# cb-geo/2d-lbm-dem

Measured on AMD Instinct MI355X. Metric: MLUPS (D2Q9 collide+stream, coupled LBM-DEM step) on 4096^2 / 50k grains, higher is better.
Workload: dtype f64; 1 GPU; 4096x4096 D2Q9 MRT + 50000 grains (synthetic row packing, seed 1234); lx=4096, ly=4096, grains=50000, npDEM=12, step=1 fluid step + npDEM DEM sub-steps (+ Verlet rebuild every 100 DEM steps), force_kernel=parity, fused_launches_reading_one_map=1996, settle_steps=40, decomposition=none

## Files before the change

2d-lbm-dem_amd/csrc/lbm_fused.hip:

```cpp


#include "lbm_march.h"
#include <type_traits>

#ifdef LBMDEM_AB
void launch_march3_ab(int which, int lx_template, const real* fin, real* fout, const int* obst_old, const int* obst_new,
                      const LatticeView& L, const GrainFluidView& G, const ForceSlots& S, int nstrips, int nwork, int remap,
                      int seg_rows, int seg_stride, int grid, hipStream_t st);
#endif

namespace {

template <int TX, int TY>
struct TileCtx {
  const Tile<TX, TY>& T;
  const LatticeView& L;
  const GrainFluidView& G;
  int px, py, gx, gy;
  __device__ __forceinline__ real own(int q) const { return T.F(q, px, py); }
  __device__ __forceinline__ real in(int d) const { return T.F(OPPq(d), px + EXq(d), py + EYq(d)); }
  __device__ __forceinline__ int o_own() const { return T.O(px, py); }
  __device__ __forceinline__ int o_nb(int d) const { return T.O(px + EXq(d), py + EYq(d)); }
  __device__ __forceinline__ bool act_nb(int d) const {
    return T.active(L, G, px + EXq(d), py + EYq(d), gx + EXq(d), gy + EYq(d));
  }
  __device__ __forceinline__ GP gp_nb(int d) const { return load_gp(G, o_nb(d)); }
};

template <int TX, int TY>
__global__ __launch_bounds__(256) void k_collide_stream(const real* __restrict__ fin,
                                                        real* __restrict__ fout,
                                                        const int* __restrict__ ob_old,
                                                        const int* __restrict__ ob_new, LatticeView L,
                                                        GrainFluidView G, int tiles_y, int ntiles,
                                                        int xcd_remap) {
  LBMDEM_GATE(L.gate);
  using TT = Tile<TX, TY>;
  __shared__ real sF[9 * TT::RX * TT::RY];
  __shared__ int sO[TT::OX * TT::OY];
  TT T{sF, sO};
  const int tid = threadIdx.x;
  int t = blockIdx.x;
  if (xcd_remap) {
    const int per = gridDim.x >> 3;
    t = (t & 7) * per + (t >> 3);
  }
  if (t >= ntiles) return;
  const int ty0 = (t % tiles_y) * TY;
  const int txl0 = L.xo0 + (t / tiles_y) * TX;

  for (int k = tid; k < TT::OX * TT::OY; k += 256) {
    const int ox = k / TT::OY, oy = k % TT::OY;
    const int xl = txl0 - 2 + ox, y = ty0 - 2 + oy;
    int v = L.n;
    if (xl >= 0 && xl < L.nxl && y >= 0 && y < L.ly) v = ob_new[(long)xl * L.sy + y];
    sO[k] = v;
  }
  __syncthreads();

  for (int k = tid; k < TT::RX * TT::RY; k += 256) {
    const int rx = k / TT::RY, ry = k % TT::RY;
    const int xl = txl0 - 1 + rx, y = ty0 - 1 + ry;
    if (xl < 0 || xl >= L.nxl || y < 0 || y >= L.ly) continue;
    const int gx = L.gx0 + xl;
    const long node = (long)xl * L.sy + y;
    const bool interior = gx >= 1 && gx <= L.lx - 2 && y >= 1 && y <= L.ly - 2;
    real f[9];
    const int oo = interior ? ob_old[node] : -1;
    if (oo != -1) {
      grain_equilibrium(L, load_gp(G, oo), gx, y, f);
    } else {
#pragma unroll
      for (int q = 0; q < 9; ++q) f[q] = fin[fidx(q, node)];
    }
    if (interior && sO[(rx + 1) * TT::OY + (ry + 1)] == -1) mrt_collide(L, f);
#pragma unroll
    for (int q = 0; q < 9; ++q) sF[(q * TT::RX + rx) * TT::RY + ry] = f[q];
  }
  __syncthreads();

  for (int k = tid; k < TX * TY; k += 256) {
    const int px = k / TY, py = k % TY;
    const int xl = txl0 + px, gy = ty0 + py;
    if (xl >= L.xo1 || gy >= L.ly) continue;
    const int gx = L.gx0 + xl;
    const long node = (long)xl * L.sy + gy;
    const TileCtx<TX, TY> C{T, L, G, px, py, gx, gy};
    fout[fidx(0, node)] = T.F(0, px, py);
    fout[fidx(1, node)] = pull_one<1>(C, L, G, gx, gy);
    fout[fidx(2, node)] = pull_one<2>(C, L, G, gx, gy);
    fout[fidx(3, node)] = pull_one<3>(C, L, G, gx, gy);
    fout[fidx(4, node)] = pull_one<4>(C, L, G, gx, gy);
    fout[fidx(5, node)] = pull_one<5>(C, L, G, gx, gy);
    fout[fidx(6, node)] = pull_one<6>(C, L, G, gx, gy);
    fout[fidx(7, node)] = pull_one<7>(C, L, G, gx, gy);
    fout[fidx(8, node)] = pull_one<8>(C, L, G, gx, gy);
  }
}

struct MarchPlan {
  int nlev, band_rows, chunk;
  int seg[4];
  int off[4];
  int first[5];
};

constexpr int LINK_SLOTS = 64;

template <int WW, bool CHG, bool EDGE>
__device__ __forceinline__ void march_item(const real* __restrict__ fin, real* __restrict__ fout,
                                           const int* __restrict__ ob_old, const int* __restrict__ ob_new,
                                           const LatticeView& L, const LatticeView& Lk, const GrainFluidView& G,
                                           const ForceSlots& S, const ObstChange& CH, int strip, int xs, int xe,
                                           const RecRing ring,
                                           real* const pay, int* const desc, int lane, int w) {
  (void)w;
  constexpr int OFF = (64 - WW) / 2;
  const int y = strip * WW - OFF + lane;
  const bool yin = !EDGE || (y >= 0 && y < L.ly);
  const bool writer = lane >= OFF && lane < OFF + WW && yin;
  const bool deep_y = !EDGE || (strip * WW >= 2 && strip * WW + WW - 1 <= L.ly - 3);

  auto row_ok = [&](int xl) { return !EDGE || (yin && xl >= 0 && xl < L.nxl); };
  const int ycl = !EDGE ? y : (y < 0 ? 0 : (y >= L.ly ? L.ly - 1 : y));
  unsigned long long cm = ~0ull;
  const int row0 = __builtin_amdgcn_readfirstlane(xs - 2 < 0 ? 0 : xs - 2);
  const int frow = L.sy * 9 * (int)sizeof(real), irow = L.sy * 4;
  const __amdgpu_buffer_rsrc_t fin_rs = make_rs(fin + (long)row0 * L.sy * 9, (long)(L.nxl - row0) * frow);
  const __amdgpu_buffer_rsrc_t fout_rs = make_rs(fout + (long)row0 * L.sy * 9, (long)(L.nxl - row0) * frow);
  const __amdgpu_buffer_rsrc_t id_rs = make_rs(ob_new + (long)row0 * L.sy, (long)(L.nxl - row0) * irow);
  const __amdgpu_buffer_rsrc_t old_rs = make_rs(ob_old + (long)row0 * L.sy, (long)(L.nxl - row0) * irow);
  const int fcol = fcol_bytes(ycl), icol = ycl * 4;
  auto rel_row = [&](int xl) { return (xl < 0 ? 0 : (xl >= L.nxl ? L.nxl - 1 : xl)) - row0; };
  if (CHG) {
    const int r0 = xs - 1, first = r0 < 0 ? 0 : r0;
    const unsigned* wp = CH.bits + (long)strip * CH.words + (first >> 5);
    const unsigned w0 = __builtin_amdgcn_readfirstlane(wp[0]), w1 = __builtin_amdgcn_readfirstlane(wp[1]);
    const unsigned w2 = __builtin_amdgcn_readfirstlane(wp[2]);
    const int sh = __builtin_amdgcn_readfirstlane(first & 31);
    cm = (unsigned long long)w0 | ((unsigned long long)w1 << 32);
    if (sh) cm = (cm >> sh) | ((unsigned long long)w2 << (64 - sh));
    if (r0 < 0) cm <<= 1;
  }
  auto load_old = [&](int xl, int same) -> int {
    if (!CHG) return __builtin_amdgcn_raw_buffer_load_b32(old_rs, icol, rel_row(xl) * irow, 0);
    const int keep = (cm & 1ull) ? 0 : -1;
    cm = (cm >> 1) | (1ull << 63);
    const int v = __builtin_amdgcn_raw_buffer_load_b32(old_rs, (rel_row(xl) * irow + icol) | (keep & (int)0x80000000), 0, 0);
    return v | (same & keep);
  };
  auto load_id = [&](int xl) -> int {
    const int v = __builtin_amdgcn_raw_buffer_load_b32(id_rs, icol, rel_row(xl) * irow, 0);
    if (!EDGE) return v;
    return (xl >= 0 && xl < L.nxl && ycl == y) ? v : L.n;
  };
  auto load_raw = [&](int xl, real (&raw)[9]) {
    const int so = rel_row(xl) * frow;
    raw[0] = buf_load_real<0 * F_QBYTES>(fin_rs, fcol, so); raw[1] = buf_load_real<1 * F_QBYTES>(fin_rs, fcol, so);
    raw[2] = buf_load_real<2 * F_QBYTES>(fin_rs, fcol, so); raw[3] = buf_load_real<3 * F_QBYTES>(fin_rs, fcol, so);
    raw[4] = buf_load_real<4 * F_QBYTES>(fin_rs, fcol, so); raw[5] = buf_load_real<5 * F_QBYTES>(fin_rs, fcol, so);
    raw[6] = buf_load_real<6 * F_QBYTES>(fin_rs, fcol, so); raw[7] = buf_load_real<7 * F_QBYTES>(fin_rs, fcol, so);
    raw[8] = buf_load_real<8 * F_QBYTES>(fin_rs, fcol, so);
  };
  auto interior = [&](int xl) {
    const int gx = L.gx0 + xl;
    return !EDGE || (row_ok(xl) && gx >= 1 && gx <= L.lx - 2 && y >= 1 && y <= L.ly - 2);
  };
  auto make_fstar = [&](int xl, real (&f)[9], int oo, const GPv& g, int on) {
    const bool in = interior(xl);
    if (in && oo != -1) grain_equilibrium(L, g, L.gx0 + xl, y, f);
    if (in && on == -1) mrt_collide(L, f);
  };
  auto grain_rec = [&](int id) { return load_gp(G, (id < 0 || id >= L.n) ? 0 : id); };
  auto reinit_rec = [&](int id) { return load_gpv(G, (id < 0 || id >= L.n) ? 0 : id); };

  real Fm[9], F0[9], Fp[9], bufA[9], bufB[9];

  const int iA = load_id(xs - 2);
  int iB = load_id(xs - 1);
  int iC = load_id(xs);
  int iD = load_id(xs + 1);
  int iE = load_id(xs + 2);
  {
    int oo = load_old(xs - 1, iB);
    load_raw(xs - 1, Fm);
    make_fstar(xs - 1, Fm, oo, reinit_rec(oo), iB);
    oo = load_old(xs, iC);
    load_raw(xs, F0);
    make_fstar(xs, F0, oo, reinit_rec(oo), iC);
  }
  ring.put(xs - 1, lane, grain_rec(iB), iB);
  ring.put(xs, lane, grain_rec(iC), iC);
  ring.put(xs + 1, lane, grain_rec(iD), iD);
  ring.put(xs + 2, lane, grain_rec(iE), iE);
  int inext = load_id(xs + 3);
  int oo1 = load_old(xs + 1, iD);
  int oo2 = load_old(xs + 2, iE);
  GP rec_next = grain_rec(inext);
  GPv gv_next = ring.getv(xs + 1, lane);
  load_raw(xs + 1, bufA);
  load_raw(xs + 2, bufB);
  auto sol_of = [&](int c) -> lmask { return __ballot(c != -1); };
  auto hmax_of = [&](int c) { const int m = dpp_up1(c), p = dpp_dn1(c), t = m > c ? m : c; return t > p ? t : p; };
  auto act_of = [&](lmask sa, lmask sb, lmask sc, int hma, int hmb, int hmc, int a, int b, int c, int xl, int ycol) -> lmask {
    const lmask enclosed = sb & m_enclosed(sa, sb, sc);
    lmask act = sb & ~enclosed;
    const int t = hma > hmb ? hma : hmb;
    const lmask rare = __ballot((t > hmc ? t : hmc) > b) & enclosed;
    if (rare != 0) {
      const bool on = node_active(L, G, ids3_of(a), ids3_of(b), ids3_of(c), L.gx0 + xl, ycol, [&] { return ring.get(xl, lane); });
      act |= __ballot(on) & rare;
    }
    return act;
  };
  lmask solB = sol_of(iB), solC = sol_of(iC), solD = sol_of(iD), solE = sol_of(iE);
  int hmC = hmax_of(iC), hmD = hmax_of(iD), hmE = hmax_of(iE);
  lmask actM = act_of(sol_of(iA), solB, solC, hmax_of(iA), hmax_of(iB), hmC, iA, iB, iC, xs - 1, y);
  lmask act0 = act_of(solB, solC, solD, hmax_of(iB), hmC, hmD, iB, iC, iD, xs, y);
  const lmask wmask = EDGE ? __ballot(writer) : (((lmask)1 << WW) - 1) << OFF;

  auto iterate = [&](int x, real (&buf)[9]) {
#pragma unroll
    for (int q = 0; q < 9; ++q) Fp[q] = buf[q];
    {
      const bool in = interior(x + 1), re = in && oo1 != -1, moved = re && oo1 != iD;
      GPv g = gv_next;
      asm volatile("" : "+v"(g.x1), "+v"(g.x2), "+v"(g.v1), "+v"(g.v2), "+v"(g.v3));
      if (__ballot(moved) != 0) {
        if (moved) g = reinit_rec(oo1);
      }
      if (re) grain_equilibrium(Lk, g, L.gx0 + x + 1, y, Fp);
      if (in && iD == -1) mrt_collide(Lk, Fp);
    }
    const int iF = inext;
    oo1 = oo2;
    inext = load_id(x + 4);
    oo2 = load_old(x + 3, iF);
    __builtin_amdgcn_sched_barrier(0);
    load_raw(x + 3 < xe ? x + 3 : xe, buf);
    __builtin_amdgcn_sched_barrier(0);
    int y_act = y;
    asm volatile("" : "+v"(y_act));
    const lmask actP = act_of(solC, solD, solE, hmC, hmD, hmE, iC, iD, iE, x + 1, y_act);

    real Fo[9], In[9];
#pragma unroll
    for (int q = 0; q < 9; ++q) Fo[q] = F0[q];
    In[0] = 0.0;
    In[2] = Fm[6];
    In[6] = Fp[2];
    In[1] = shfl_dn1z(Fm[5]);
    In[8] = shfl_dn1z(F0[4]);
    In[7] = shfl_dn1z(Fp[3]);
    In[3] = shfl_up1z(Fm[7]);
    In[4] = shfl_up1z(F0[8]);
    In[5] = shfl_up1z(Fp[1]);
    {
      const int gx = L.gx0 + x;
      const int so_row = (x - row0) * frow;
      const bool deep = !EDGE || (deep_y && gx >= 2 && gx <= L.lx - 3);
      const lmask wm = x < xe ? wmask : 0;
#define MARCH_SRC(Q) m_at<-EYq(Q)>(MARCH_ROW(-EXq(Q), solB, solC, solD))
#define MARCH_LINK(Q) (wm & ~solC & MARCH_SRC(Q))
#define MARCH_HAZ(Q) (Q <= 4 ? MARCH_LINK(Q) & m_at<EYq(Q)>(MARCH_ROW(EXq(Q), solB, solC, solD)) : 0)
#define MARCH_RESET(Q) (solC & MARCH_SRC(Q) & m_at<-EYq(Q)>(MARCH_ROW(-EXq(Q), actM, act0, actP)))
      unsigned ibb = 0, nnm = 0, hzm = 0;
      int T = 0;
      if (deep) {
        T = __popcll(MARCH_LINK(1)) + __popcll(MARCH_LINK(2)) + __popcll(MARCH_LINK(3)) + __popcll(MARCH_LINK(4)) +
            __popcll(MARCH_LINK(5)) + __popcll(MARCH_LINK(6)) + __popcll(MARCH_LINK(7)) + __popcll(MARCH_LINK(8));
      } else if constexpr (EDGE) {
        RegCtx C;
        C.ring = ring;
        C.row = x;
        C.lane = lane;
#pragma unroll
        for (int q = 0; q < 9; ++q) { C.Fo[q] = Fo[q]; C.In[q] = In[q]; }
        const Ids3 b3 = ids3_of(iB), c3 = ids3_of(iC), d3 = ids3_of(iD);
        C.o0 = iC;
        C.onb[0] = 0;
        C.onb[1] = b3.p; C.onb[2] = b3.c; C.onb[3] = b3.m; C.onb[4] = c3.m;
        C.onb[5] = d3.m; C.onb[6] = d3.c; C.onb[7] = d3.p; C.onb[8] = c3.p;
        C.act = 0;
#define MARCH_ACTBIT(D) C.act |= lane_of(m_at<EYq(D)>(MARCH_ROW(EXq(D), actM, act0, actP))) ? 1u << D : 0u;
        MARCH_ACTBIT(1) MARCH_ACTBIT(2) MARCH_ACTBIT(3) MARCH_ACTBIT(4) MARCH_ACTBIT(5) MARCH_ACTBIT(6) MARCH_ACTBIT(7) MARCH_ACTBIT(8)
#undef MARCH_ACTBIT
        if (writer && x < xe) classify_store_row<true>(C, L, gx, y, fout, fbase_xy(L, x, y), ibb, nnm, hzm);
#pragma unroll
        for (int q = 1; q < 9; ++q) T += __popcll(__ballot((ibb >> q) & 1u));
      }
      const bool merged = deep && T <= LINK_SLOTS;
      auto store_row = [&](auto with_results) {
        if (lane_of(wm)) {
          buf_store_real<0>(Fo[0], fout_rs, fcol, so_row);
          real res[9];
          if constexpr (decltype(with_results)::value) {
            int before = 0;
#define MARCH_RES(Q)                                                                               \
            {                                                                                      \
              const lmask b = MARCH_LINK(Q);                                                       \
              res[Q] = pay[((before + (int)mbcnt(b)) & (LINK_SLOTS - 1)) * 4];                     \
              before += __popcll(b);                                                               \
            }
            MARCH_RES(1) MARCH_RES(2) MARCH_RES(3) MARCH_RES(4) MARCH_RES(5) MARCH_RES(6) MARCH_RES(7) MARCH_RES(8)
#undef MARCH_RES
          }
#define MARCH_STORE(Q)                                                                             \
          {                                                                                        \
            real v = lane_of(MARCH_RESET(Q)) ? Wq(Q) : In[OPPq(Q)];                                \
            if constexpr (decltype(with_results)::value) v = lane_of(MARCH_LINK(Q)) ? res[Q] : v;  \
            buf_store_real<Q * F_QBYTES>(v, fout_rs, fcol, so_row);                                \
          }
          MARCH_STORE(1) MARCH_STORE(2) MARCH_STORE(3) MARCH_STORE(4) MARCH_STORE(5) MARCH_STORE(6) MARCH_STORE(7) MARCH_STORE(8)
#undef MARCH_STORE
        }
      };
      if (deep && !merged) store_row(std::false_type{});
      for (int base = 0; base < T; base += LINK_SLOTS) {
        int before = 0;
        if (deep) {
#define MARCH_COMPACT(Q)                                                                           \
          {                                                                                        \
            const lmask b = MARCH_LINK(Q);                                                         \
            const int t = before + (int)mbcnt(b) - base;                                           \
            before += __popcll(b);                                                                 \
            if (lane_of(b) && (unsigned)t < (unsigned)LINK_SLOTS) {                                \
              desc[t] = lane | (Q << 8) | (1 << 12) | (lane_of(MARCH_HAZ(Q)) ? 1 << 13 : 0);       \
              pay[t * 4 + 0] = Fo[OPPq(Q)];                                                        \
              pay[t * 4 + 1] = Fo[Q];                                                              \
              pay[t * 4 + 2] = In[Q];                                                              \
              pay[t * 4 + 3] = In[OPPq(Q)];                                                        \
            }                                                                                      \
          }
          MARCH_COMPACT(1) MARCH_COMPACT(2) MARCH_COMPACT(3) MARCH_COMPACT(4)
          MARCH_COMPACT(5) MARCH_COMPACT(6) MARCH_COMPACT(7) MARCH_COMPACT(8)
#undef MARCH_COMPACT
        } else if constexpr (EDGE) {
#pragma unroll
          for (int q = 1; q < 9; ++q) {
            const lmask b = __ballot((ibb >> q) & 1u);
            const int t = before + (int)mbcnt(b) - base;
            before += __popcll(b);
            if (((ibb >> q) & 1u) && (unsigned)t < (unsigned)LINK_SLOTS) {
              desc[t] = lane | (q << 8) | (((nnm >> q) & 1u) << 12) | (((hzm >> q) & 1u) << 13);
              pay[t * 4 + 0] = Fo[OPPq(q)];
              pay[t * 4 + 1] = Fo[q];
              pay[t * 4 + 2] = In[q];
              pay[t * 4 + 3] = In[OPPq(q)];
            }
          }
        }
        __builtin_amdgcn_wave_barrier();
        if (base + lane < T) {
          const int d = desc[lane];
          const int src = d & 63;
          RtLink k;
          k.q = (d >> 8) & 15;
          k.gx = gx;
          k.gy = y - lane + src;
          k.own_qo = pay[lane * 4 + 0];
          k.own_q = pay[lane * 4 + 1];
          k.in_q = pay[lane * 4 + 2];
          k.in_qo = pay[lane * 4 + 3];
          k.nn_int = (d >> 12) & 1;
          k.hazard = (d >> 13) & 1;
          const int ex = (k.q >= 1 && k.q <= 3) ? -1 : ((k.q >= 5 && k.q <= 7) ? 1 : 0);
          const int ey = (k.q == 1 || k.q >= 7) ? 1 : ((k.q >= 3 && k.q <= 5) ? -1 : 0);
          const GP gS = ring.get(x - ex, src - ey);
          const int owner = ring.get_id(x - ex, src - ey);
          const real out = ibb_eval_rt(Lk, k, Lk.wc_diag, Lk.wc_axis, gS, [&] { return ring.get(x + ex, src + ey); });
          if (merged) pay[lane * 4] = out;
          else buf_store_real<0>(out, fout_rs, fcol_bytes(k.gy) + k.q * F_QBYTES, so_row);
          if (S.tab != nullptr) {
            const int rel = slot_line(k.gx - ex, k.gy - ey, ex, ey, gS.xc, gS.yc) + S.half;
            if ((unsigned)rel < (unsigned)S.spd)
              S.tab[((long)owner * 8 + (k.q - 1)) * S.spd + rel] = k.own_qo + out;
          }
        }
        __builtin_amdgcn_wave_barrier();
      }
      if (merged) {
        if (T > 0) store_row(std::true_type{});
        else store_row(std::false_type{});
      }
#undef MARCH_RESET
#undef MARCH_HAZ
#undef MARCH_LINK
#undef MARCH_SRC
    }
    ring.put(x + 3, lane, rec_next, iF);
    rec_next = grain_rec(inext);
    gv_next = ring.getv(x + 2, lane);
#pragma unroll
    for (int q = 0; q < 9; ++q) { Fm[q] = F0[q]; F0[q] = Fp[q]; }
    iB = iC; iC = iD; iD = iE; iE = iF;
    solB = solC; solC = solD; solD = solE; solE = sol_of(iF);
    hmC = hmD; hmD = hmE; hmE = hmax_of(iF);
    actM = act0; act0 = actP;
  };

  for (int x = xs; x < xe; x += 2) {
    iterate(x, bufA);
    iterate(x + 1, bufB);
  }
}

constexpr int WPB = 4;

template <int LX, int MINW, int WW, bool CHG = false>
__global__ __launch_bounds__(64 * WPB, MINW) void k_cs_march(const real* __restrict__ fin, real* __restrict__ fout,
                                                  const int* __restrict__ ob_old,
                                                  const int* __restrict__ ob_new, LatticeView L,
                                                  GrainFluidView G, ForceSlots S, int nstrips, int nwork,
                                                  int xcd_remap, int seg_rows, int seg_stride, MarchPlan P, ObstChange CH) {
  LBMDEM_GATE(L.gate);
  const int lane = threadIdx.x & 63;
  int blk = blockIdx.x;
  int w, strip, xs, rows_per_wave;
  if (LX == 0 && P.nlev > 0) {
    const int band = blk & 7, local = (blk >> 3) * WPB + (threadIdx.x >> 6);
    if (local >= P.first[P.nlev]) return;
    int l = 0;
#pragma unroll
    for (int k = 1; k < 4; ++k)
      if (k < P.nlev && local >= P.first[k]) l = k;
    const int j = local - P.first[l], sg = j / nstrips;
    strip = j - sg * nstrips;
    rows_per_wave = P.seg[l];
    const int v = P.off[l] + sg * rows_per_wave, c = v / P.chunk;
    xs = L.xo0 + (c * 8 + band) * P.chunk + (v - c * P.chunk);
    if (xs >= L.xo1) return;
    w = band * P.first[P.nlev] + local;
  } else {
    if (xcd_remap) {
      const int per = gridDim.x >> 3;
      blk = (blk & 7) * per + (blk >> 3);
    }
    w = blk * WPB + (threadIdx.x >> 6);
    if (w >= nwork) return;
    const int seg = w / nstrips;
    strip = w - seg * nstrips;
    rows_per_wave = LX > 0 ? LX : seg_rows;
    xs = L.xo0 + seg * seg_stride;
  }
  strip = __builtin_amdgcn_readfirstlane(strip);
  xs = __builtin_amdgcn_readfirstlane(xs);
  const int xe = __builtin_amdgcn_readfirstlane(xs + rows_per_wave < L.xo1 ? xs + rows_per_wave : L.xo1);
  __shared__ real2 sRec[WPB * REC_RING * 4 * 64];
  __shared__ int sRid[WPB * REC_RING * 64];
  const RecRing ring{sRec + (threadIdx.x >> 6) * (REC_RING * 4 * 64), sRid + (threadIdx.x >> 6) * (REC_RING * 64)};
  __shared__ real sPay[WPB * LINK_SLOTS * 4];
  __shared__ int sDesc[WPB * LINK_SLOTS];
  real* const pay = sPay + (threadIdx.x >> 6) * (LINK_SLOTS * 4);
  int* const desc = sDesc + (threadIdx.x >> 6) * LINK_SLOTS;
  __shared__ LatticeView sLat[WPB];
  LatticeView* const Lk = sLat + (threadIdx.x >> 6);
  if (lane == 0) *Lk = L;
  __builtin_amdgcn_wave_barrier();
  constexpr int OFF = (64 - WW) / 2;
  const int y_lo = strip * WW - OFF;
  const bool inner = y_lo >= 1 && y_lo + 63 <= L.ly - 2 && L.gx0 + xs >= 2 && L.gx0 + xe <= L.lx - 2 && xs >= 2 &&
                     xe + 2 <= L.nxl;
  if (inner) march_item<WW, CHG, false>(fin, fout, ob_old, ob_new, L, *Lk, G, S, CH, strip, xs, xe, ring, pay, desc, lane, w);
  else march_item<WW, CHG, true>(fin, fout, ob_old, ob_new, L, *Lk, G, S, CH, strip, xs, xe, ring, pay, desc, lane, w);
}

}


template <int TX, int TY>
static void launch_cs(const real* fin, real* fout, const int* obst_old, const int* obst_new,
                      const LatticeView& L, const GrainFluidView& G, int remap, hipStream_t st) {
  const int rows = L.xo1 - L.xo0;
  const int tiles_y = (L.ly + TY - 1) / TY, tiles_x = (rows + TX - 1) / TX;
  const int ntiles = tiles_y * tiles_x;
  const int grid = remap ? ((ntiles + 7) / 8) * 8 : ntiles;
  hipLaunchKernelGGL((k_collide_stream<TX, TY>), dim3(grid), dim3(256), 0, st, fin, fout, obst_old, obst_new,
                     L, G, tiles_y, ntiles, remap);
}

static int march_segment_rows(int rows, int nstrips) {
  const int resident = 256 * 2 * 4;
  int nseg = (2 * resident + nstrips - 1) / nstrips;
  if (nseg < 1) nseg = 1;
  int seg_rows = rows / nseg;
  seg_rows &= ~1;
  if (seg_rows < 8) seg_rows = 8;
  if (seg_rows > 32) seg_rows = 32;
  return seg_rows;
}

static MarchPlan march_plan(int rows, int nstrips, int main_seg, const int (*tail)[2], int ntail, int chunk) {
  MarchPlan P{};
  if (rows < 8 * (main_seg + 64)) return P;
  if (chunk <= 0) chunk = 1 << 30;
  int band_rows = (((rows + 7) / 8) + 7) & ~7;
  if (chunk < band_rows) band_rows = (band_rows + chunk - 1) / chunk * chunk;
  else chunk = band_rows;
  P.chunk = chunk;
  int tail_rows = 0;
  for (int k = 0; k < ntail; ++k) tail_rows += tail[k][1];
  if (band_rows - tail_rows < main_seg) return P;
  const int main_rows = (band_rows - tail_rows) / main_seg * main_seg;
  int rem = band_rows - tail_rows - main_rows;
  P.band_rows = band_rows;
  int off = 0, first = 0, lev = 0;
  bool fits = true;
  auto add = [&](int seg, int r) {
    if (r <= 0) return;
    if (chunk % seg != 0 || off % seg != 0) fits = false;
    P.seg[lev] = seg; P.off[lev] = off; P.first[lev] = first;
    off += r; first += r / seg * nstrips; ++lev;
  };
  add(main_seg, main_rows);
  for (int k = 0; k < ntail; ++k) {
    int r = tail[k][1];
    const int seg = tail[k][0];
    const int take = k + 1 < ntail ? rem / seg * seg : rem;
    r += take; rem -= take;
    add(seg, r);
  }
  if (rem != 0 || !fits) return MarchPlan{};
  P.nlev = lev;
  P.first[lev] = first;
  return P;
}

static constexpr bool plan_level_ok(int seg, int rows) { return seg >= 8 && seg % 8 == 0 && rows % seg == 0; }

static MarchPlan product_plan(int rows, int nstrips, int seg_rows) {
  if (seg_rows < 32) return MarchPlan{};
  constexpr int main_seg = 64, ntail = 3, chunk = 64;
  static constexpr int tail[ntail][2] = {{32, 64}, {16, 64}, {8, 64}};
  static_assert(plan_level_ok(main_seg, chunk), "a chunk of a band holds whole main segments");
  static_assert(plan_level_ok(tail[0][0], tail[0][1]) && plan_level_ok(tail[1][0], tail[1][1]) &&
                    plan_level_ok(tail[2][0], tail[2][1]),
                "every tail level is cut into whole segments");
  return march_plan(rows, nstrips, main_seg, tail, ntail, chunk);
}

#ifdef LBMDEM_AB
static int cs_variant() {
  static int v = -1;
  if (v < 0) {
    const char* e = getenv("LBMDEM_CS_VARIANT");
    v = e ? atoi(e) : 25;
  }
  return v;
}
static int march_kernel() {
  static const int v = getenv("LBMDEM_MARCH") ? atoi(getenv("LBMDEM_MARCH")) : 2;
  return v;
}
#endif

constexpr int MARCH_WW = 60;

template <int LX, int MINW, int WW = MARCH_WW>
static void launch_march(const real* fin, real* fout, const int* obst_old, const int* obst_new,
                         const LatticeView& L, const GrainFluidView& G, const ForceSlots& S, int remap,
                         hipStream_t st, ObstChange chg = ObstChange{nullptr, 0, 0, 0}) {
  const int rows = L.xo1 - L.xo0;
  const int nstrips = (L.ly + WW - 1) / WW;
  if (chg.ww != WW || chg.off != (64 - WW) / 2) chg = ObstChange{nullptr, 0, 0, 0};
  int seg_rows = LX;
  if (LX == 0) {
    seg_rows = march_segment_rows(rows, nstrips);
  }
  const int nseg = (rows + seg_rows - 1) / seg_rows;
  int nwork = nstrips * nseg;
  int grid = (nwork + WPB - 1) / WPB;
  if (remap) grid = ((grid + 7) / 8) * 8;
  MarchPlan P{};
  if (LX == 0 && remap) P = product_plan(rows, nstrips, seg_rows);
  if (P.nlev > 0) {
    nwork = 8 * P.first[P.nlev];
    grid = 8 * ((P.first[P.nlev] + WPB - 1) / WPB);
  }
#ifdef LBMDEM_AB
  if constexpr (WW == 62) {
    const int mk = march_kernel();
    if (mk == 21 || mk == 22) {
      launch_march3_ab(mk, LX, fin, fout, obst_old, obst_new, L, G, S, nstrips, nwork, remap, seg_rows, seg_rows, grid, st);
      return;
    }
  }
#endif
  if (LX == 0 && chg.bits != nullptr) {
    hipLaunchKernelGGL((k_cs_march<LX, MINW, WW, LX == 0>), dim3(grid), dim3(64 * WPB), 0, st, fin, fout, obst_old, obst_new, L, G,
                       S, nstrips, nwork, remap, seg_rows, seg_rows, P, chg);
    return;
  }
  hipLaunchKernelGGL((k_cs_march<LX, MINW, WW>), dim3(grid), dim3(64 * WPB), 0, st, fin, fout, obst_old, obst_new, L, G,
                     S, nstrips, nwork, remap, seg_rows, seg_rows, P, chg);
}

static void launch_march_two_ranges(const real* fin, real* fout, const int* obst_old, const int* obst_new,
                                    const LatticeView& L, const GrainFluidView& G, const ForceSlots& S, int lo0, int w,
                                    int hi0, hipStream_t st) {
  constexpr int WW = MARCH_WW;
  LatticeView Ls = L;
  Ls.xo0 = lo0; Ls.xo1 = hi0 + w;
  const int nstrips = (L.ly + WW - 1) / WW;
  const int nwork = nstrips * 2;
  const int grid = (nwork + WPB - 1) / WPB;
  hipLaunchKernelGGL((k_cs_march<0, 2, WW>), dim3(grid), dim3(64 * WPB), 0, st, fin, fout, obst_old, obst_new, Ls, G, S, nstrips,
                     nwork, 0, w, hi0 - lo0, MarchPlan{}, ObstChange{nullptr, 0, 0, 0});
}

bool collide_stream_fills_slots(const LatticeView& L) { return L.reduced_lt1 != 0; }

void collide_stream_work_order(const LatticeView& L, int* info) {
  for (int k = 0; k < 12; ++k) info[k] = 0;
  if (!L.reduced_lt1) return;
  const int rows = L.xo1 - L.xo0, nstrips = (L.ly + MARCH_WW - 1) / MARCH_WW;
  const int seg_rows = march_segment_rows(rows, nstrips);
  const MarchPlan P = product_plan(rows, nstrips, seg_rows);
  info[0] = P.nlev;
  if (P.nlev == 0) {
    info[3] = seg_rows;
    info[7] = rows;
    info[11] = nstrips * ((rows + seg_rows - 1) / seg_rows);
    return;
  }
  info[1] = P.band_rows; info[2] = P.chunk;
  for (int l = 0; l < P.nlev; ++l) {
    info[3 + l] = P.seg[l];
    info[7 + l] = (l + 1 < P.nlev ? P.off[l + 1] : P.band_rows) - P.off[l];
  }
  info[11] = 8 * P.first[P.nlev];
}

void collide_stream_windows(int* ww, int* off) { *ww = MARCH_WW; *off = (64 - MARCH_WW) / 2; }

void launch_collide_stream(const real* fin, real* fout, const int* obst_old, const int* obst_new,
                           const LatticeView& L, const GrainFluidView& G, const ForceSlots& S, hipStream_t st,
                           const ObstChange& chg) {
#ifdef LBMDEM_AB
  if (getenv("LBMDEM_CS_VARIANT") && L.reduced_lt1) {
    const int v = cs_variant(), remap = (v >> 3) & 1;
    switch (v & ~8) {
      case 16: launch_march<16, 2>(fin, fout, obst_old, obst_new, L, G, S, remap, st); return;
      case 19: launch_march<64, 2>(fin, fout, obst_old, obst_new, L, G, S, remap, st); return;
      case 20: launch_march<0, 2>(fin, fout, obst_old, obst_new, L, G, S, remap, st); return;
      case 21: launch_march<32, 2, 56>(fin, fout, obst_old, obst_new, L, G, S, remap, st); return;
      default: launch_march<32, 2>(fin, fout, obst_old, obst_new, L, G, S, remap, st); return;
    }
  }
#endif
  if (L.reduced_lt1) {
#ifdef LBMDEM_AB
    if (march_kernel() != 2) {
      launch_march<0, 2, 62>(fin, fout, obst_old, obst_new, L, G, S,  1, st);
      return;
    }
#endif
    launch_march<0, 2>(fin, fout, obst_old, obst_new, L, G, S,  1, st, chg);
  }
  else launch_cs<4, 64>(fin, fout, obst_old, obst_new, L, G, 0, st);
}

void launch_collide_stream_edges(const real* fin, real* fout, const int* obst_old, const int* obst_new,
                                 const LatticeView& L, const GrainFluidView& G, const ForceSlots& S, int lo0, int lo1,
                                 int hi0, int hi1, hipStream_t st) {
  bool one_launch = lo1 > lo0 && hi1 > hi0 && lo1 - lo0 == hi1 - hi0 && lo1 - lo0 <= 32 && lo1 <= hi0 && L.reduced_lt1;
#ifdef LBMDEM_AB
  if (getenv("LBMDEM_CS_VARIANT")) one_launch = false;
#endif
  if (one_launch) {
    launch_march_two_ranges(fin, fout, obst_old, obst_new, L, G, S, lo0, lo1 - lo0, hi0, st);
    return;
  }
  LatticeView Ls = L;
  if (lo1 > lo0) { Ls.xo0 = lo0; Ls.xo1 = lo1; launch_collide_stream(fin, fout, obst_old, obst_new, Ls, G, S, st); }
  if (hi1 > hi0) { Ls.xo0 = hi0; Ls.xo1 = hi1; launch_collide_stream(fin, fout, obst_old, obst_new, Ls, G, S, st); }
}
```

Before: 19530 MLUPS.

## Compute the next column's f-star one step ahead, overlapped with link resolution

The grain-equilibrium and MRT collision for the upcoming column move from the start of each iteration into the link-resolution loop. There they run one column ahead on the other prefetch buffer, interleaved with the LDS descriptor/payload reads, so their latency can hide behind the shared-memory and link evaluation work. The prologue now precomputes f-star for column xs+1, and the link loop becomes a do-while so the look-ahead still runs when no links exist. This raises register pressure and tightens the ordering between the two buffers, which could hurt occupancy or lead to subtle correctness issues.

```diff
diff --git a/2d-lbm-dem_amd/csrc/lbm_fused.hip b/2d-lbm-dem_amd/csrc/lbm_fused.hip
--- a/2d-lbm-dem_amd/csrc/lbm_fused.hip
+++ b/2d-lbm-dem_amd/csrc/lbm_fused.hip
@@ -188,17 +188,18 @@
     oo = load_old(xs, iC);
     load_raw(xs, F0);
     make_fstar(xs, F0, oo, reinit_rec(oo), iC);
+    oo = load_old(xs + 1, iD);
+    load_raw(xs + 1, bufA);
+    make_fstar(xs + 1, bufA, oo, reinit_rec(oo), iD);
   }
   ring.put(xs - 1, lane, grain_rec(iB), iB);
   ring.put(xs, lane, grain_rec(iC), iC);
   ring.put(xs + 1, lane, grain_rec(iD), iD);
   ring.put(xs + 2, lane, grain_rec(iE), iE);
   int inext = load_id(xs + 3);
-  int oo1 = load_old(xs + 1, iD);
   int oo2 = load_old(xs + 2, iE);
+  int oo1 = oo2;
   GP rec_next = grain_rec(inext);
-  GPv gv_next = ring.getv(xs + 1, lane);
-  load_raw(xs + 1, bufA);
   load_raw(xs + 2, bufB);
   auto sol_of = [&](int c) -> lmask { return __ballot(c != -1); };
   auto hmax_of = [&](int c) { const int m = dpp_up1(c), p = dpp_dn1(c), t = m > c ? m : c; return t > p ? t : p; };
@@ -219,19 +220,21 @@
   lmask act0 = act_of(solB, solC, solD, hmax_of(iB), hmC, hmD, iB, iC, iD, xs, y);
   const lmask wmask = EDGE ? __ballot(writer) : (((lmask)1 << WW) - 1) << OFF;
 
-  auto iterate = [&](int x, real (&buf)[9]) {
+  auto iterate = [&](int x, real (&buf)[9], real (&other)[9]) {
 #pragma unroll
     for (int q = 0; q < 9; ++q) Fp[q] = buf[q];
-    {
-      const bool in = interior(x + 1), re = in && oo1 != -1, moved = re && oo1 != iD;
+    GPv gv_next;
+    auto fstar_ahead = [&] {
+      const bool in = interior(x + 2), re = in && oo1 != -1, moved = re && oo1 != iE;
       GPv g = gv_next;
       asm volatile("" : "+v"(g.x1), "+v"(g.x2), "+v"(g.v1), "+v"(g.v2), "+v"(g.v3));
       if (__ballot(moved) != 0) {
         if (moved) g = reinit_rec(oo1);
+        asm volatile("" : "+v"(g.x1), "+v"(g.x2), "+v"(g.v1), "+v"(g.v2), "+v"(g.v3));
       }
-      if (re) grain_equilibrium(Lk, g, L.gx0 + x + 1, y, Fp);
-      if (in && iD == -1) mrt_collide(Lk, Fp);
-    }
+      if (re) grain_equilibrium(Lk, g, L.gx0 + x + 2, y, other);
+      if (in && iE == -1) mrt_collide(Lk, other);
+    };
     const int iF = inext;
     oo1 = oo2;
     inext = load_id(x + 4);
@@ -316,52 +319,63 @@
         }
       };
       if (deep && !merged) store_row(std::false_type{});
-      for (int base = 0; base < T; base += LINK_SLOTS) {
+      gv_next = ring.getv(x + 2, lane);
+      int base = 0;
+      do {
+        const bool round = base < T;
         int before = 0;
-        if (deep) {
+        if (round) {
+          if (deep) {
 #define MARCH_COMPACT(Q)                                                                           \
-          {                                                                                        \
-            const lmask b = MARCH_LINK(Q);                                                         \
-            const int t = before + (int)mbcnt(b) - base;                                           \
-            before += __popcll(b);                                                                 \
-            if (lane_of(b) && (unsigned)t < (unsigned)LINK_SLOTS) {                                \
-              desc[t] = lane | (Q << 8) | (1 << 12) | (lane_of(MARCH_HAZ(Q)) ? 1 << 13 : 0);       \
-              pay[t * 4 + 0] = Fo[OPPq(Q)];                                                        \
-              pay[t * 4 + 1] = Fo[Q];                                                              \
-              pay[t * 4 + 2] = In[Q];                                                              \
-              pay[t * 4 + 3] = In[OPPq(Q)];                                                        \
-            }                                                                                      \
-          }
-          MARCH_COMPACT(1) MARCH_COMPACT(2) MARCH_COMPACT(3) MARCH_COMPACT(4)
-          MARCH_COMPACT(5) MARCH_COMPACT(6) MARCH_COMPACT(7) MARCH_COMPACT(8)
+            {                                                                                        \
+              const lmask b = MARCH_LINK(Q);                                                         \
+              const int t = before + (int)mbcnt(b) - base;                                           \
+              before += __popcll(b);                                                                 \
+              if (lane_of(b) && (unsigned)t < (unsigned)LINK_SLOTS) {                                \
+                desc[t] = lane | (Q << 8) | (1 << 12) | (lane_of(MARCH_HAZ(Q)) ? 1 << 13 : 0);       \
+                pay[t * 4 + 0] = Fo[OPPq(Q)];                                                        \
+                pay[t * 4 + 1] = Fo[Q];                                                              \
+                pay[t * 4 + 2] = In[Q];                                                              \
+                pay[t * 4 + 3] = In[OPPq(Q)];                                                        \
+              }                                                                                      \
+            }
+            MARCH_COMPACT(1) MARCH_COMPACT(2) MARCH_COMPACT(3) MARCH_COMPACT(4)
+            MARCH_COMPACT(5) MARCH_COMPACT(6) MARCH_COMPACT(7) MARCH_COMPACT(8)
 #undef MARCH_COMPACT
-        } else if constexpr (EDGE) {
-#pragma unroll
-          for (int q = 1; q < 9; ++q) {
-            const lmask b = __ballot((ibb >> q) & 1u);
-            const int t = before + (int)mbcnt(b) - base;
-            before += __popcll(b);
-            if (((ibb >> q) & 1u) && (unsigned)t < (unsigned)LINK_SLOTS) {
-              desc[t] = lane | (q << 8) | (((nnm >> q) & 1u) << 12) | (((hzm >> q) & 1u) << 13);
-              pay[t * 4 + 0] = Fo[OPPq(q)];
-              pay[t * 4 + 1] = Fo[q];
-              pay[t * 4 + 2] = In[q];
-              pay[t * 4 + 3] = In[OPPq(q)];
+          } else if constexpr (EDGE) {
+#pragma unroll
+            for (int q = 1; q < 9; ++q) {
+              const lmask b = __ballot((ibb >> q) & 1u);
+              const int t = before + (int)mbcnt(b) - base;
+              before += __popcll(b);
+              if (((ibb >> q) & 1u) && (unsigned)t < (unsigned)LINK_SLOTS) {
+                desc[t] = lane | (q << 8) | (((nnm >> q) & 1u) << 12) | (((hzm >> q) & 1u) << 13);
+                pay[t * 4 + 0] = Fo[OPPq(q)];
+                pay[t * 4 + 1] = Fo[q];
+                pay[t * 4 + 2] = In[q];
+                pay[t * 4 + 3] = In[OPPq(q)];
+              }
             }
           }
+          __builtin_amdgcn_wave_barrier();
         }
-        __builtin_amdgcn_wave_barrier();
-        if (base + lane < T) {
-          const int d = desc[lane];
+        const int d = desc[lane];
+        const real p0 = pay[lane * 4 + 0], p1 = pay[lane * 4 + 1], p2 = pay[lane * 4 + 2], p3 = pay[lane * 4 + 3];
+        if (base == 0) {
+          __builtin_amdgcn_sched_barrier(0);
+          fstar_ahead();
+          __builtin_amdgcn_sched_barrier(0);
+        }
+        if (round && base + lane < T) {
           const int src = d & 63;
           RtLink k;
           k.q = (d >> 8) & 15;
           k.gx = gx;
           k.gy = y - lane + src;
-          k.own_qo = pay[lane * 4 + 0];
-          k.own_q = pay[lane * 4 + 1];
-          k.in_q = pay[lane * 4 + 2];
-          k.in_qo = pay[lane * 4 + 3];
+          k.own_qo = p0;
+          k.own_q = p1;
+          k.in_q = p2;
+          k.in_qo = p3;
           k.nn_int = (d >> 12) & 1;
           k.hazard = (d >> 13) & 1;
           const int ex = (k.q >= 1 && k.q <= 3) ? -1 : ((k.q >= 5 && k.q <= 7) ? 1 : 0);
@@ -378,7 +392,8 @@
           }
         }
         __builtin_amdgcn_wave_barrier();
-      }
+        base += LINK_SLOTS;
+      } while (base < T);
       if (merged) {
         if (T > 0) store_row(std::true_type{});
         else store_row(std::false_type{});
@@ -390,7 +405,6 @@
     }
     ring.put(x + 3, lane, rec_next, iF);
     rec_next = grain_rec(inext);
-    gv_next = ring.getv(x + 2, lane);
 #pragma unroll
     for (int q = 0; q < 9; ++q) { Fm[q] = F0[q]; F0[q] = Fp[q]; }
     iB = iC; iC = iD; iD = iE; iE = iF;
@@ -400,8 +414,8 @@
   };
 
   for (int x = xs; x < xe; x += 2) {
-    iterate(x, bufA);
-    iterate(x + 1, bufB);
+    iterate(x, bufA, bufB);
+    iterate(x + 1, bufB, bufA);
   }
 }
 
```

New measurement: 19220 MLUPS. 0.984x the previous value.
